# simochen/flowtrack.pytorch

Measured on AMD Instinct MI355X. Metric: pose crops/sec (ResNet-50 + 3-deconv head, 256x192), higher is better.
Workload: dtype fp16; 1 GPU; ResNet-50 pose head fp16, batch 64 x 256x192 synthetic crops per GPU (BASELINE.json configs[1]); per_gpu_batch=64, resident_batches=4, parallelism=dp1: batch sharded, one process per GPU

## Files before the change

flowtrack/pytorch_amd/_lib.py:

```python
from __future__ import annotations

import ctypes
import os
from ctypes import POINTER, c_char_p, c_double, c_float, c_int, c_int32, c_uint64, c_void_p

HERE = os.path.dirname(os.path.abspath(__file__))
LIB_PATH = os.environ.get("FT_LIB_PATH") or os.path.join(HERE, "libflowtrack_hip.so")

FT_OK = 0
FT_ERR_INVALID_ARG = 1
FT_ERR_UNSUPPORTED = 2
FT_F16, FT_F32 = 0, 1
FT_ACT_NONE, FT_ACT_RELU, FT_ACT_LEAKY = 0, 1, 2
FT_LAYOUT_NHWC, FT_LAYOUT_NCHW_F32 = 0, 1
FT_RGB_MEAN_SPLITS = 64


class FlowtrackHipError(RuntimeError):
    pass


class ConvDesc(ctypes.Structure):

    _fields_ = [
# ... 43 lines not shown
    "ft_memcpy_async": (c_int, [c_void_p, c_void_p, ctypes.c_size_t, c_void_p]),
    "ft_conv_pack_geometry": (c_int, [POINTER(ConvDesc), POINTER(ConvGeometry)]),
    "ft_conv_tile_candidates": (c_int, [POINTER(ConvDesc), POINTER(c_int), c_int]),
    "ft_conv_workspace_bytes": (ctypes.c_size_t, [POINTER(ConvDesc)]),
    "ft_conv2d_fwd_ws": (c_int, [POINTER(ConvDesc), c_void_p, c_void_p, c_void_p, c_void_p, c_void_p, c_void_p, c_void_p,
                                 ctypes.c_size_t, c_void_p]),
    "ft_conv_tap_source": (c_int, [POINTER(ConvDesc), c_int, c_int, c_int, POINTER(c_int), POINTER(c_int)]),
    "ft_conv2d_fwd": (c_int, [POINTER(ConvDesc), c_void_p, c_void_p, c_void_p, c_void_p, c_void_p,
                              c_void_p, c_void_p]),
    "ft_conv_flops": (c_double, [POINTER(ConvDesc)]),
    "ft_conv_direct_supported": (c_int, [POINTER(ConvDesc)]),
    "ft_conv_direct_stream_id": (c_int, [POINTER(ConvDesc)]),
    "ft_conv_direct_weight_bytes": (ctypes.c_longlong, [POINTER(ConvDesc)]),
    "ft_conv_direct_pack": (c_int, [POINTER(ConvDesc), c_void_p, c_int, c_int, c_void_p, c_void_p]),
    "ft_conv_direct_fwd": (c_int, [POINTER(ConvDesc), c_void_p, c_void_p, c_void_p, c_void_p, c_void_p, c_void_p, c_void_p]),
    "ft_bottleneck_supported": (c_int, [POINTER(BottleneckDesc)]),
    "ft_bottleneck_fwd": (c_int, [POINTER(BottleneckDesc), c_void_p, c_void_p, c_void_p, c_void_p, c_void_p, c_void_p, c_void_p]),
    "ft_bottleneck_flops": (c_double, [POINTER(BottleneckDesc)]),
    "ft_bottleneck_rstat_supported": (c_int, [POINTER(BottleneckDesc)]),
    "ft_bottleneck_rstat_weight_bytes": (ctypes.c_longlong, []),
    "ft_bottleneck_rstat_fwd": (c_int, [POINTER(BottleneckDesc), c_void_p, c_void_p, c_void_p, c_void_p]),
    "ft_bottleneck_stream_supported": (c_int, [POINTER(BottleneckDesc)]),
    "ft_bottleneck_stream_folds": (c_int, [POINTER(BottleneckDesc)]),
    "ft_bottleneck_stream_weight_bytes": (ctypes.c_longlong, [POINTER(BottleneckDesc)]),
    "ft_bottleneck_stream_pack": (c_int, [POINTER(BottleneckDesc), c_void_p, c_void_p, c_void_p, c_void_p, c_void_p]),
    "ft_bottleneck_stream_fwd": (c_int, [POINTER(BottleneckDesc), c_void_p, c_void_p, c_void_p, c_void_p, c_void_p]),
    "ft_pack_nchw_to_nhwc": (c_int, [c_void_p, c_void_p] + [c_int] * 8 + [c_void_p]),
    "ft_unpack_nhwc_to_nchw": (c_int, [c_void_p, c_void_p, c_int, c_int, c_int, c_int, c_int, c_int, c_int,
                                       c_void_p]),
    "ft_maxpool3x3s2_fwd": (c_int, [c_void_p, c_void_p, c_int, c_int, c_int, c_int, c_int, c_void_p]),
    "ft_bn_batch_stats": (c_int, [c_void_p, c_int, c_int, c_int, c_int, c_int, c_int, c_void_p, c_void_p, c_void_p, c_void_p]),
    "ft_heatmap_max_preds": (c_int, [c_void_p, c_int, c_int, c_int, c_int, c_int, c_void_p, c_void_p, c_void_p,
                                     c_void_p]),
    "ft_heatmap_keypoint_rows": (c_int, [c_void_p, c_int, c_int, c_int, c_int, c_int, c_void_p, c_void_p, c_void_p]),
    "ft_heatmap_min_margin": (c_int, [c_void_p, c_int, c_int, c_int, c_int, c_void_p, c_void_p]),
    "ft_heatmap_argmax_screen": (c_int, [c_void_p, c_int, c_int, c_int, c_int, c_float, c_void_p, c_void_p, c_void_p]),
    "ft_flow_rgb_mean": (c_int, [c_void_p, c_int, c_int, c_int, c_void_p, c_void_p, c_void_p]),
    "ft_flow_pack_pair": (c_int, [c_void_p, c_void_p, c_float, c_void_p] + [c_int] * 7 + [c_void_p]),
    "ft_flow_mean_pack_pair_state_words": (ctypes.c_longlong, [c_int, c_int, c_int]),
    "ft_flow_pack_pair_sums_chunks": (ctypes.c_longlong, [c_int]),
    "ft_conv_shift_nstride_supported": (c_int, [POINTER(ConvDesc)]),
    "ft_flow_pack_pair_sums": (c_int, [c_void_p, c_float, c_void_p] + [c_int] * 6 + [c_void_p, c_void_p]),
    "ft_flow_mean_fold": (c_int, [c_void_p, c_float, c_void_p] + [c_int] * 6 + [c_void_p, c_void_p, c_void_p, c_int, c_void_p, c_void_p,
                                  c_void_p]),
    "ft_flow_mean_pack_pair": (c_int, [c_void_p, c_float, c_void_p, c_int, c_int, c_void_p, c_int, c_int] + [c_int] * 4
                               + [c_void_p, c_void_p, c_void_p]),
# ... 65 lines not shown
```

flowtrack/pytorch_amd/csrc/bottleneck_stream.hip:

```cpp
#include <stdlib.h>

#include <type_traits>

#include "ft_common.h"

namespace ft {
namespace {

struct BnsParams {
  const char* x;
  char* y;
  const char* ws;
  const char* tab;
  int H, W, TH;
  int ppi, total;
  int TWc, csplit;
  int Ho, Wo;
  int x_cstride, x_coff, y_cstride, y_coff;
  unsigned x_bytes, y_bytes, ws_bytes;
  int dbg;
};

template <int N, int I = 0, typename F>
__device__ __forceinline__ void bns_unroll(F&& f) {
// ... 697 lines not shown
#pragma unroll
      for (int e = 0; e < 6; ++e)
#pragma unroll
        for (int i = 0; i < CTW; ++i)
          shp[e][i] = __builtin_amdgcn_raw_buffer_load_b32(rsrc_t, so, 4 * (e * P + (CTW * wcol + i) * 32), 0);
    } else {
#pragma unroll
      for (int t = 0; t < 48 / NW; ++t)
        __builtin_amdgcn_raw_ptr_buffer_load_lds(rsrc_t, (lds_ptr)(smem + TABS + (t * NW + wave) * 256), 4, (unsigned)lane * 4u, (t * NW + wave) * 256, 0, 0);
    }
  };
  [[maybe_unused]] auto add_shift = [&](int e, auto& A, auto mtc) {
    constexpr int MT = decltype(mtc)::value;
#pragma unroll
    for (int i = 0; i < CTW; ++i) {
      const uint4_t sa = uint4_t{shp[e][i], 0u, 0u, 0u};
#pragma unroll
      for (int j = 0; j < MT; ++j)
        A[i][j] = __builtin_amdgcn_mfma_f32_32x32x16_f16(__builtin_bit_cast(half8_t, sa), __builtin_bit_cast(half8_t, onesB), A[i][j], 0, 0, 0);
    }
  };
  issue_x(0, 0);
  load_a(std::integral_constant<int, 0>{}, 0);
  issue_touch();
  load_tables();
  asm volatile("" ::: "memory");
  issue_x(1, 1);
  issue_x(2, 2);
  bns_unroll<D - 1>([&](auto sc) { load_a(std::integral_constant<int, decltype(sc)::value + 1>{}, decltype(sc)::value + 1); });
  if (tid < ROWB / 16) *reinterpret_cast<uint4_t*>(smem + ZROW + tid * 16) = uint4_t{0u, 0u, 0u, 0u};

  uint4_t res[4][CTW][MT2][2];
  int m_out[MT2], hp_out[MT2];
#pragma unroll
  for (int j = 0; j < MT2; ++j) {
    m_out[j] = j * 32 + l31;
    if constexpr (XH) {
      const int r = m_out[j] / TWc;
      hp_out[j] = (r + 1) * PW + (m_out[j] - r * TWc) + 1;
    } else if constexpr (HEAD) {
      const int r = m_out[j] / TWc;
      hp_out[j] = (2 * r + 1) * W + 2 * (m_out[j] - r * TWc);
    } else {
      hp_out[j] = m_out[j] + W;
    }
  }

  float16_t acc1[CTW][MT1];
#pragma unroll
// ... 372 lines not shown
      zero_acc();
      if constexpr (!WSTG) {
        asm volatile("s_waitcnt lgkmcnt(0)" ::: "memory");
        BNS_BARRIER();
      } else {
        asm volatile("" ::: "memory");
      }
      readout(qc);
    });
  }
  if (p.dbg & 32) {
    ts[5] = __builtin_amdgcn_s_memtime();
    asm volatile("s_waitcnt vmcnt(0)" ::: "memory");
    ts[6] = __builtin_amdgcn_s_memtime();
    if (tid == 0) {
      unsigned long long* o = reinterpret_cast<unsigned long long*>(p.y + ((size_t)((n * p.H + y0) * W) * p.y_cstride + p.y_coff) * 2);
#pragma unroll
      for (int i = 0; i < 8; ++i) o[i] = ts[i];
    }
  }
#endif
}

template <int P>
__global__ __launch_bounds__(256) void bns_pack_kernel(const half_t* __restrict__ w1, const half_t* __restrict__ w2,
                                                       const half_t* __restrict__ w3, uint4_t* __restrict__ out) {
  using G = BnsGeom<P>;
  const int idx = blockIdx.x * 256 + threadIdx.x;
  if (idx >= G::GEND * G::WSTEP / 16) return;
  const int lane = idx & 63, frag = idx >> 6;
  const int per_step = 4 * G::NCT;
  const int g = frag / per_step, f = frag - g * per_step;
  const int kk = f / G::NCT, i = f - kk * G::NCT;
  const int l31 = lane & 31, lhi = lane >> 5;
  const int co_t = 32 * i + bns_sigma(l31);
  const int k_t = 16 * kk + 8 * lhi;
  const half_t* src;
  if (g < G::G2) {
    src = w1 + (size_t)co_t * G::C + 64 * g + k_t;
  } else if (g < G::G3) {
    const int s = g - G::G2, tap = s / G::KC, kc = s - tap * G::KC;
    src = w2 + (size_t)co_t * (9 * P) + tap * P + 64 * kc + k_t;
  } else {
    const int s = g - G::G3, q = s / G::KC, kc = s - q * G::KC;
    src = w3 + (size_t)(q * P + co_t) * P + 64 * kc + k_t;
  }
  out[idx] = *reinterpret_cast<const uint4_t*>(src);
}

__global__ __launch_bounds__(256) void bns_pack_head_kernel(const half_t* __restrict__ w1, const half_t* __restrict__ w2,
                                                            uint4_t* __restrict__ out, int C) {
  using G = BnsGeom<256>;
  const int nc1 = C / 64, gend = nc1 + 9 * G::KC;
  const int idx = blockIdx.x * 256 + threadIdx.x;
  if (idx >= gend * G::WSTEP / 16) return;
  const int lane = idx & 63, frag = idx >> 6;
  const int per_step = 4 * G::NCT;
  const int g = frag / per_step, f = frag - g * per_step;
  const int kk = f / G::NCT, i = f - kk * G::NCT;
  const int l31 = lane & 31, lhi = lane >> 5;
  const int co_t = 32 * i + bns_sigma(l31);
  const int k_t = 16 * kk + 8 * lhi;
  const half_t* src;
  if (g < nc1) {
    src = w1 + (size_t)co_t * C + 64 * g + k_t;
  } else {
    const int sft = g - nc1, tap = sft / G::KC, kc = sft - tap * G::KC;
    src = w2 + (size_t)co_t * (9 * 256) + tap * 256 + 64 * kc + k_t;
  }
  out[idx] = *reinterpret_cast<const uint4_t*>(src);
}

// ... 43 lines not shown
    auto cost = [&](int th, int mt1, int mt2) {
      const long long wg = (long long)d->N * ceil_div(d->H, th);
      return ((wg + 255) / 256) * (long long)(32 * mt1 + 104 * mt2);
    };
    bool small = th_b < 1 || (th_s >= 1 && cost(th_s, 3, 2) < cost(th_b, 4, 3));
    if (force128 == 1 && th_b >= 1) small = false;
    if (force128 == 2 && th_s >= 1) small = true;
    const int th = small ? th_s : th_b;
    *out = BnsPlan{small ? 5 : 0, th, ceil_div(d->H, th), d->W, 1};
    return FT_OK;
  }
  const int th_big = rows(96, 120), th_small = rows(64, 96);
  int xs = 0, x_tw = 0, x_th = 0;
  for (int cs = 2; cs <= 4 && !xs; ++cs) {
    const int tw = ceil_div(d->W, cs);
    int th = 32 / tw;
    const int th2 = 64 / (tw + 2) - 2;
    th = th < th2 ? th : th2;
    if (th < 1 || tw * (cs - 1) >= d->W) continue;
    th = th < d->H ? th : d->H;
    xs = cs; x_tw = tw; x_th = ceil_div(d->H, ceil_div(d->H, th));
  }
  if (th_big < 1 && th_small < 1 && !xs) return FT_ERR_UNSUPPORTED;
  int pick;
  if (force == 1 || force == 2 || (force == 3 && xs)) pick = force;
  else {
    auto cost = [&](int th, int mt1, int mt2) {
      const long long wg = (long long)d->N * ceil_div(d->H, th);
      return ((wg + 255) / 256) * (long long)(64 * mt1 + 208 * mt2);
    };
    if (th_big < 1) pick = 2;
    else if (th_small < 1) pick = 1;
    else pick = cost(th_big, 4, 3) <= cost(th_small, 3, 2) ? 1 : 2;
    if (pick == 1 && th_big < 1) pick = 2;
    if (pick == 2 && th_small < 1) pick = th_big >= 1 ? 1 : 3;
    if (xs && pick != 3) {
      const long long wgx = (long long)d->N * ceil_div(d->H, x_th) * xs;
      const long long cx = ((wgx + 255) / 256) * (long long)(64 * 2 + 208 * 1);
      const long long cf = pick == 1 ? cost(th_big, 4, 3) : cost(th_small, 3, 2);
      if (cx < cf) pick = 3;
    }
  }
  if (pick == 1 && th_big < 1) pick = 2;
  if (pick == 2 && th_small < 1) pick = th_big >= 1 ? 1 : 3;
  if (pick == 3) {
    *out = BnsPlan{3, x_th, ceil_div(d->H, x_th) * xs, x_tw, xs};
    return FT_OK;
  }
  const int th = pick == 1 ? th_big : th_small;
  *out = BnsPlan{pick, th, ceil_div(d->H, th), d->W, 1};
  return FT_OK;
}

template <int P, int MT1, int MT2, bool FOLD = false>
static int bns_launch(const BnsParams& p, hipStream_t s) {
  auto k = bottleneck_stream_kernel<P, MT1, MT2, FOLD>;
  static bool attr_done[64] = {};
  int dev = 0;
  FT_HIP_CHECK(hipGetDevice(&dev));
  if (dev < 0 || dev >= 64 || !attr_done[dev]) {
    FT_HIP_CHECK(hipFuncSetAttribute(reinterpret_cast<const void*>(k), hipFuncAttributeMaxDynamicSharedMemorySize, BnsGeom<P>::LDS_BYTES));
    if (dev >= 0 && dev < 64) attr_done[dev] = true;
  }
  hipLaunchKernelGGL(k, dim3(p.total), dim3(256), BnsGeom<P>::LDS_BYTES, s, p);
// ... 3 lines not shown

#ifndef FT_BNS_SLOTS
#define FT_BNS_SLOTS 4
#endif
#ifndef FT_BNS_XH_SLOTS
#define FT_BNS_XH_SLOTS 3
#endif
template <int MT1, int MT2, bool XH, int HEADC = 0, int NW = 4, bool FOLD = false>
static int bns_launch_direct(const BnsParams& p, hipStream_t s) {
  auto k = bottleneck_stream_direct_kernel<MT1, MT2, XH, XH ? FT_BNS_XH_SLOTS : FT_BNS_SLOTS, HEADC, NW, FOLD>;
  constexpr int lds = 81920 + 2 * MT2 * 32 * 512;
  static bool attr_done[64] = {};
  int dev = 0;
  FT_HIP_CHECK(hipGetDevice(&dev));
  if (dev < 0 || dev >= 64 || !attr_done[dev]) {
    FT_HIP_CHECK(hipFuncSetAttribute(reinterpret_cast<const void*>(k), hipFuncAttributeMaxDynamicSharedMemorySize, lds));
    if (dev >= 0 && dev < 64) attr_done[dev] = true;
  }
  hipLaunchKernelGGL(k, dim3(p.total), dim3(64 * NW), lds, s, p);
  FT_LAUNCH_CHECK("bottleneck_stream_direct_kernel");
  return FT_OK;
}

}
}

extern "C" int ft_bottleneck_stream_supported(const ft_bottleneck_desc* d) {
  ft::BnsPlan pl;
  return ft::bns_plan(d, &pl);
}

extern "C" int ft_bottleneck_stream_folds(const ft_bottleneck_desc* d) {
  ft::BnsPlan pl;
  if (ft::bns_plan(d, &pl) != FT_OK) return 0;
  return pl.variant != 4;
}

extern "C" long long ft_bottleneck_stream_weight_bytes(const ft_bottleneck_desc* d) {
  ft::BnsPlan pl;
  if (ft::bns_plan(d, &pl) != FT_OK) return 0;
  if (pl.variant == 4) return (long long)(d->C / 64 + 9 * ft::BnsGeom<256>::KC) * ft::BnsGeom<256>::WSTEP;
  return d->P == 128 ? (long long)ft::BnsGeom<128>::GEND * ft::BnsGeom<128>::WSTEP : (long long)ft::BnsGeom<256>::GEND * ft::BnsGeom<256>::WSTEP;
}

extern "C" int ft_bottleneck_stream_pack(const ft_bottleneck_desc* d, const void* w1, const void* w2, const void* w3, void* wstream,
                                         ft_stream_t stream) {
  using namespace ft;
  BnsPlan pl;
  const int st = bns_plan(d, &pl);
  if (st != FT_OK) return st;
  if (!w1 || !w2 || (!w3 && pl.variant != 4) || !wstream) return FT_ERR_INVALID_ARG;
  hipStream_t s = as_stream(stream);
  const half_t *a = static_cast<const half_t*>(w1), *b = static_cast<const half_t*>(w2), *c = static_cast<const half_t*>(w3);
  if (pl.variant == 4) {
    const int n16 = (int)(ft_bottleneck_stream_weight_bytes(d) / 16);
    hipLaunchKernelGGL(bns_pack_head_kernel, dim3(ceil_div(n16, 256)), dim3(256), 0, s, a, b, static_cast<uint4_t*>(wstream), d->C);
    FT_LAUNCH_CHECK("bns_pack_head_kernel");
    return FT_OK;
  }
  if (d->P == 128) {
    const int n16 = BnsGeom<128>::GEND * BnsGeom<128>::WSTEP / 16;
    hipLaunchKernelGGL(bns_pack_kernel<128>, dim3(ceil_div(n16, 256)), dim3(256), 0, s, a, b, c, static_cast<uint4_t*>(wstream));
  } else {
    const int n16 = BnsGeom<256>::GEND * BnsGeom<256>::WSTEP / 16;
    hipLaunchKernelGGL(bns_pack_kernel<256>, dim3(ceil_div(n16, 256)), dim3(256), 0, s, a, b, c, static_cast<uint4_t*>(wstream));
  }
  FT_LAUNCH_CHECK("bns_pack_kernel");
  return FT_OK;
}

extern "C" int ft_bottleneck_stream_fwd(const ft_bottleneck_desc* d, const void* x, const void* wstream, const float* tables, void* y,
                                        ft_stream_t stream) {
  using namespace ft;
  BnsPlan pl;
  const int st = bns_plan(d, &pl);
  if (st != FT_OK) return st;
  if (!x || !wstream || !tables || !y || x == y) return FT_ERR_INVALID_ARG;
  if (d->folded && pl.variant == 4) return FT_ERR_UNSUPPORTED;
  BnsParams p{};
  p.x = static_cast<const char*>(x);
  p.y = static_cast<char*>(y);
  p.ws = static_cast<const char*>(wstream);
  p.tab = reinterpret_cast<const char*>(tables);
  p.H = d->H; p.W = d->W; p.TH = pl.TH; p.ppi = pl.ppi;
  p.TWc = pl.TWc; p.csplit = pl.csplit;
  if (pl.variant == 4) { p.Ho = d->H / 2; p.Wo = d->W / 2; }
  p.total = d->N * pl.ppi;
  p.x_cstride = d->x_cstride; p.x_coff = d->x_coff; p.y_cstride = d->y_cstride; p.y_coff = d->y_coff;
  p.x_bytes = (unsigned)((size_t)d->N * d->H * d->W * d->x_cstride * 2);
  p.y_bytes = (unsigned)((size_t)d->N * d->H * d->W * d->y_cstride * 2);
  p.ws_bytes = (unsigned)ft_bottleneck_stream_weight_bytes(d);
  if (pl.variant == 4) p.y_bytes = (unsigned)((size_t)d->N * p.Ho * p.Wo * d->y_cstride * 2);
  static const int dbg = dev_env_int("FT_BNS_DBG", 0);
  p.dbg = dbg;
  if (dbg & 64) p.ws_bytes = 0;
  if (dbg & 128) p.x_bytes = 0;
  hipStream_t s = as_stream(stream);
  const bool waves8 = dev_env_int("FT_BNS_WAVES", pl.variant == 3 ? 8 : 4) == 8;
  if (d->folded) {
    switch (pl.variant) {
      case 0: return bns_launch<128, 4, 3, true>(p, s);
      case 5: return bns_launch<128, 3, 2, true>(p, s);
      case 1: return bns_launch<256, 4, 3, true>(p, s);
      case 3: return waves8 ? bns_launch_direct<2, 1, true, 0, 8, true>(p, s) : bns_launch_direct<2, 1, true, 0, 4, true>(p, s);
      default: return waves8 ? bns_launch_direct<3, 2, false, 0, 8, true>(p, s) : bns_launch_direct<3, 2, false, 0, 4, true>(p, s);
    }
  }
  switch (pl.variant) {
    case 0: return bns_launch<128, 4, 3>(p, s);
    case 5: return bns_launch<128, 3, 2>(p, s);
    case 1: return bns_launch<256, 4, 3>(p, s);
    case 3: return waves8 ? bns_launch_direct<2, 1, true, 0, 8>(p, s) : bns_launch_direct<2, 1, true>(p, s);
    case 4: return waves8 ? bns_launch_direct<4, 1, false, 8, 8>(p, s) : bns_launch_direct<4, 1, false, 8>(p, s);
    default:
      return waves8 ? bns_launch_direct<3, 2, false, 0, 8>(p, s) : bns_launch_direct<3, 2, false>(p, s);
  }
}
```

flowtrack/pytorch_amd/csrc/ft_common.h:

```cpp
#pragma once
#include <hip/hip_runtime.h>
#include <stdint.h>
#include <stdlib.h>

#include "flowtrack_hip.h"

namespace ft {

int record_hip_error(hipError_t e, const char* what);

#define FT_HIP_CHECK(expr)                                         \
  do {                                                             \
    hipError_t _e = (expr);                                        \
    if (_e != hipSuccess) return ::ft::record_hip_error(_e, #expr); \
  } while (0)

#define FT_LAUNCH_CHECK(name)                                        \
  do {                                                               \
    hipError_t _e = hipGetLastError();                               \
    if (_e != hipSuccess) return ::ft::record_hip_error(_e, name);   \
  } while (0)

#define FT_RAISE_LDS(kernel, bytes)                                                                              \
  do {                                                                                                           \
// ... 51 lines not shown
  }
}
__device__ __forceinline__ half8_t bn_res_relu_acc8(const float16_t& acc, int h, const float4_t (&sc)[4], const float4_t (&sh)[4], const half8_t& rs) {
  half8_t o;
#pragma unroll
  for (int e = 0; e < 8; e += 2) {
    const int r = h * 8 + e;
    const half2_t v = bn_res_relu_pk(acc[r], acc[r + 1], sc[r >> 2][r & 3], sc[r >> 2][(r & 3) + 1], sh[r >> 2][r & 3], sh[r >> 2][(r & 3) + 1], rs[e], rs[e + 1]);
    o[e] = v[0];
    o[e + 1] = v[1];
  }
  return o;
}

__device__ __forceinline__ void relu_acc16(const float16_t& acc, half8_t (&h8)[2]) {
#pragma unroll
  for (int r = 0; r < 16; r += 2) {
    const half2_t o = __builtin_elementwise_max(__builtin_convertvector(float2_t{acc[r], acc[r + 1]}, half2_t), half2_t{(half_t)0.f, (half_t)0.f});
    h8[r >> 3][r & 7] = o[0];
    h8[r >> 3][(r & 7) + 1] = o[1];
  }
}

#ifndef FT_YSTORE_AUX
#define FT_YSTORE_AUX 16
#endif
#define FT_YSTORE_BUF_AUX (FT_YSTORE_AUX == 2 ? 2 : ((FT_YSTORE_AUX & 16) ? FT_YSTORE_AUX : 0))
__device__ __forceinline__ void store_out16(void* ptr, uint4_t v) {
#if FT_YSTORE_AUX == 16
  asm volatile("global_store_dwordx4 %0, %1, off sc1\n\ts_nop 1" ::"v"(ptr), "v"(v) : "memory");
#elif FT_YSTORE_AUX == 17
  asm volatile("global_store_dwordx4 %0, %1, off sc0 sc1\n\ts_nop 1" ::"v"(ptr), "v"(v) : "memory");
#elif FT_YSTORE_AUX == 2
  __builtin_nontemporal_store(v, reinterpret_cast<uint4_t*>(ptr));
#else
  *reinterpret_cast<uint4_t*>(ptr) = v;
#endif
}

}
```

flowtrack/pytorch_amd/hip_ops.py:

```python
from __future__ import annotations

import ctypes
import functools
import json
import os
import sys
from dataclasses import dataclass
from typing import List, Optional, Sequence, Tuple

import torch

from . import _lib
from ._lib import (FT_ACT_LEAKY, FT_ACT_NONE, FT_ACT_RELU, FT_LAYOUT_NCHW_F32, FT_LAYOUT_NHWC,
                   ConvDesc, ConvGeometry, FlowtrackHipError, check)

ACT_CODES = {None: FT_ACT_NONE, "none": FT_ACT_NONE, "relu": FT_ACT_RELU, "leaky": FT_ACT_LEAKY}


def require_gpu(device: torch.device) -> None:
    if device.type != "cuda" or not torch.cuda.is_available():
        raise FlowtrackHipError(
            "the flowtrack HIP path needs a ROCm GPU (model.cuda()); there is no CPU fallback — "
            "use oracle/ for CPU reference results")

# ... 1018 lines not shown
    if scale is not None:
        w = w * scale[:, None]
    return w.half().contiguous(), (shift if shift is not None else torch.zeros(conv.cout))


def _fold_representable(convs) -> bool:
    for c in convs:
        w, sh = _folded_kmajor(c)
        if not bool(torch.isfinite(w.float()).all()) or not bool(torch.isfinite(sh.float().half().float()).all()):
            return False
    return True


def shift_pairs(shift: torch.Tensor) -> torch.Tensor:
    hi = shift.float().half()
    lo = (shift.float() - hi.float()).half()
    return torch.stack([hi, lo], dim=-1).contiguous().view(torch.int32).reshape(-1)


def _bottleneck_stream_operands(c1: "FusedConv", d, x: ActView, planes: int, p1, p2, p3, convs=None):
    lib = _lib.load()
    (w1, s1, b1), (w2, s2, b2), (w3, s3, b3) = p1, p2, p3
    folded = convs is not None
    key = ("bns_stream_folded" if folded else "bns_stream", x.N, x.H, x.W)
    cached = c1._packed.get(key) if hasattr(c1, "_packed") else None
    if cached is None:
        P = planes
        if folded:
            dev = x.t.device
            (w1, sh1), (w2, sh2), (w3, sh3) = (_folded_kmajor(c) for c in convs)
            if (tuple(w1.shape), tuple(w2.shape), tuple(w3.shape)) != ((P, 4 * P), (P, 9 * P), (4 * P, P)):
                raise FlowtrackHipError(f"folded bottleneck weights: unexpected shapes {tuple(w1.shape)} {tuple(w2.shape)} {tuple(w3.shape)}")
            w1, w2, w3 = w1.to(dev), w2.to(dev), w3.to(dev)
            tables = torch.cat([shift_pairs(sh1), shift_pairs(sh2), shift_pairs(sh3)]).contiguous().to(dev)
        else:
            tables = torch.cat([s1.flatten()[:P], b1.flatten()[:P], s2.flatten()[:P], b2.flatten()[:P]] +
                               [t.flatten()[q * P:(q + 1) * P] for q in range(4) for t in (s3, b3)]).float().contiguous()
        nbytes = int(lib.ft_bottleneck_stream_weight_bytes(ctypes.byref(d)))
        wstream = torch.empty(nbytes, dtype=torch.uint8, device=x.t.device)
        check(lib.ft_bottleneck_stream_pack(ctypes.byref(d), w1.data_ptr(), w2.data_ptr(), w3.data_ptr(), wstream.data_ptr(),
                                            current_stream_handle(x.t.device)), "ft_bottleneck_stream_pack")
        torch.cuda.current_stream(x.t.device).synchronize()
        cached = (wstream, tables)
        if hasattr(c1, "_packed"):
            c1._packed[key] = cached
    return cached

# ... 146 lines not shown
```

include/flowtrack_hip.h:

```cpp
#ifndef FLOWTRACK_HIP_H_
#define FLOWTRACK_HIP_H_

#include <stddef.h>
#include <stdint.h>

#ifdef __cplusplus
extern "C" {
#endif

enum {
  FT_OK = 0,
  FT_ERR_INVALID_ARG = 1,
  FT_ERR_UNSUPPORTED = 2,
  FT_ERR_HIP = 3,
  FT_ERR_NO_DEVICE = 4
};

enum { FT_F16 = 0, FT_F32 = 1 };
enum { FT_ACT_NONE = 0, FT_ACT_RELU = 1, FT_ACT_LEAKY = 2 };
enum { FT_LAYOUT_NHWC = 0, FT_LAYOUT_NCHW_F32 = 1 };

typedef void* ft_stream_t;

int ft_version(void);
// ... 70 lines not shown
int ft_conv_direct_pack(const ft_conv_desc* d, const void* w_packed, int kpad, int cout_pad, void* wstream, ft_stream_t stream);
int ft_conv_direct_fwd(const ft_conv_desc* d, const void* x, const void* wstream, const float* scale, const float* shift,
                       const void* residual, void* y, ft_stream_t stream);

typedef struct ft_bottleneck_desc {
  int dtype;
  int N, H, W;
  int C, P;
  int x_cstride, x_coff;
  int y_cstride, y_coff;
  int head_only;
  int projection;
  int stride;
  int folded;
} ft_bottleneck_desc;
int ft_bottleneck_supported(const ft_bottleneck_desc* d);
int ft_bottleneck_fwd(const ft_bottleneck_desc* d, const void* x,
                      const void* w1, const void* w2, const void* w3,
                      const float* scale_shift, void* y, ft_stream_t stream);
double ft_bottleneck_flops(const ft_bottleneck_desc* d);

int ft_bottleneck_stream_supported(const ft_bottleneck_desc* d);
int ft_bottleneck_stream_folds(const ft_bottleneck_desc* d);
long long ft_bottleneck_stream_weight_bytes(const ft_bottleneck_desc* d);
int ft_bottleneck_stream_pack(const ft_bottleneck_desc* d, const void* w1, const void* w2, const void* w3, void* wstream,
                              ft_stream_t stream);
int ft_bottleneck_stream_fwd(const ft_bottleneck_desc* d, const void* x, const void* wstream, const float* tables, void* y,
                             ft_stream_t stream);

int ft_pack_nchw_to_nhwc(const float* x, void* y, int N, int C, int H, int W,
                         int cpad, int lpad, int wpitch, int dtype,
                         ft_stream_t stream);
int ft_unpack_nhwc_to_nchw(const void* x, float* y, int N, int C, int H, int W,
                           int x_cstride, int x_coff, int dtype,
                           ft_stream_t stream);
int ft_maxpool3x3s2_fwd(const void* x, void* y, int N, int Hi, int Wi, int C,
                        int dtype, ft_stream_t stream);

int ft_bn_batch_stats(const void* x, int N, int H, int W, int C, int x_cstride, int dtype,
                      float* workspace, float* mean, float* var, ft_stream_t stream);

int ft_heatmap_max_preds(const float* heatmaps, int N, int K, int H, int W,
                         int adjust_coords, int32_t* idx, float* score,
                         float* coords, ft_stream_t stream);
int ft_heatmap_keypoint_rows(const float* heatmaps, int N, int K, int H, int W,
                             int adjust_coords, int32_t* idx, float* rows,
// ... 99 lines not shown
```

Baseline: 56140 crops/s.

## Add 16x16 MFMA tile variant of fused bottleneck stream kernel for P=256

Adds a new fused bottleneck kernel variant for P=256 folded blocks that uses 16x16x32 MFMA tiles with smaller pixel tiles (48-80 rows-worth), plus a matching weight-pack kernel and a packed-weight layout key so cached weights match the chosen variant. The planner picks this variant when its estimated wave cost beats the existing 32x32 variants, aiming to reduce tile-quantization waste and improve workgroup balance on the late ResNet stage. It also inserts scheduling barriers around the prologue loads in the existing kernel. The new path adds register/LDS pressure (launch bounds 1) and relies on a heuristic cost model that may misjudge.

```diff
diff --git a/flowtrack/pytorch_amd/_lib.py b/flowtrack/pytorch_amd/_lib.py
--- a/flowtrack/pytorch_amd/_lib.py
+++ b/flowtrack/pytorch_amd/_lib.py
@@ -89,6 +89,7 @@
     "ft_bottleneck_rstat_fwd": (c_int, [POINTER(BottleneckDesc), c_void_p, c_void_p, c_void_p, c_void_p]),
     "ft_bottleneck_stream_supported": (c_int, [POINTER(BottleneckDesc)]),
     "ft_bottleneck_stream_folds": (c_int, [POINTER(BottleneckDesc)]),
+    "ft_bottleneck_stream_layout": (c_int, [POINTER(BottleneckDesc)]),
     "ft_bottleneck_stream_weight_bytes": (ctypes.c_longlong, [POINTER(BottleneckDesc)]),
     "ft_bottleneck_stream_pack": (c_int, [POINTER(BottleneckDesc), c_void_p, c_void_p, c_void_p, c_void_p, c_void_p]),
     "ft_bottleneck_stream_fwd": (c_int, [POINTER(BottleneckDesc), c_void_p, c_void_p, c_void_p, c_void_p, c_void_p]),
diff --git a/flowtrack/pytorch_amd/csrc/bottleneck_stream.hip b/flowtrack/pytorch_amd/csrc/bottleneck_stream.hip
--- a/flowtrack/pytorch_amd/csrc/bottleneck_stream.hip
+++ b/flowtrack/pytorch_amd/csrc/bottleneck_stream.hip
@@ -743,9 +743,12 @@
   };
   issue_x(0, 0);
   load_a(std::integral_constant<int, 0>{}, 0);
+  asm volatile("" ::: "memory");
+  __builtin_amdgcn_sched_barrier(0);
   issue_touch();
   load_tables();
   asm volatile("" ::: "memory");
+  __builtin_amdgcn_sched_barrier(0);
   issue_x(1, 1);
   issue_x(2, 2);
   bns_unroll<D - 1>([&](auto sc) { load_a(std::integral_constant<int, decltype(sc)::value + 1>{}, decltype(sc)::value + 1); });
@@ -1164,6 +1167,414 @@
 #endif
 }
 
+template <int NS>
+__global__ __launch_bounds__(256, 1) void bottleneck_stream_tile16_kernel(const BnsParams p) {
+#if defined(__HIP_DEVICE_COMPILE__)
+  constexpr int P = 256;
+  using G = BnsGeom<P>;
+  constexpr int NC1 = G::NC1, KC = G::KC, WSTEP = G::WSTEP, ROWB = G::ROWB;
+  constexpr int G2 = NC1, G3 = G2 + 9 * KC, GEND = G3 + 4 * KC;
+  constexpr int CT = 4, MT1 = 5, MT2 = 3, NT = 256;
+  constexpr int LX = (MT1 * 2 + 3) / 4;
+  constexpr int NOUT = MT2 * 16;
+  constexpr int ZROW = 61440, TOUCH = 77824, STG = 81920, STGB = 4 * NOUT * 128;
+  static_assert(LX * 4 * 8 * 128 <= G::XSTRIDE && MT1 * 16 * ROWB <= ZROW && STG + 2 * STGB <= 163840, "LDS map");
+  extern __shared__ __attribute__((aligned(16))) char smem[];
+  typedef __attribute__((address_space(3))) void* lds_ptr;
+  using c0 = std::integral_constant<int, 0>;
+  using c1 = std::integral_constant<int, 1>;
+  const int tid = threadIdx.x, lane = tid & 63;
+  const int wave = __builtin_amdgcn_readfirstlane(tid >> 6);
+  const int l15 = lane & 15, lq = lane >> 4;
+
+  int logical;
+  {
+    const int b = blockIdx.x;
+    const int q = p.total >> 3, r = p.total & 7, xcd = b & 7, loc = b >> 3;
+    logical = (xcd < r ? xcd * (q + 1) : r * (q + 1) + (xcd - r) * q) + loc;
+  }
+  const int n = logical / p.ppi;
+  const int W = p.W;
+  const int y0 = (logical - n * p.ppi) * p.TH;
+  const int rows_out = p.H - y0 < p.TH ? p.H - y0 : p.TH;
+  const int npix_out = rows_out * W;
+  const int npix_halo = (p.TH + 2) * W;
+  const int iy0 = y0 - 1;
+
+  const __amdgpu_buffer_rsrc_t rsrc_x = __builtin_amdgcn_make_buffer_rsrc(const_cast<char*>(p.x), 0, p.x_bytes, 0x00020000);
+  const __amdgpu_buffer_rsrc_t rsrc_y = __builtin_amdgcn_make_buffer_rsrc(p.y, 0, p.y_bytes, 0x00020000);
+  const __amdgpu_buffer_rsrc_t rsrc_w = __builtin_amdgcn_make_buffer_rsrc(const_cast<char*>(p.ws), 0, p.ws_bytes, 0x00020000);
+  const __amdgpu_buffer_rsrc_t rsrc_t = __builtin_amdgcn_make_buffer_rsrc(const_cast<char*>(p.tab), 0, (2 * P + G::C) * 4, 0x00020000);
+  constexpr unsigned kOOB = 0x80000000u;
+
+  unsigned x_voff[LX];
+#pragma unroll
+  for (int t = 0; t < LX; ++t) {
+    const int hp = (t * 4 + wave) * 8 + (lane >> 3);
+    const int hr = hp / W, hc = hp - hr * W;
+    const int iy = iy0 + hr;
+    unsigned v = kOOB;
+    if (hp < npix_halo && (unsigned)iy < (unsigned)p.H)
+      v = (unsigned)((((n * p.H + iy) * W + hc) * p.x_cstride + p.x_coff) * 2 + (((lane & 7) ^ BNS_XKEY(hp)) << 4));
+    x_voff[t] = v;
+  }
+  const unsigned lane16 = (unsigned)lane * 16u;
+  auto issue_x = [&](int c, int buf) {
+    char* dst = smem + buf * G::XSTRIDE;
+#pragma unroll
+    for (int t = 0; t < LX; ++t)
+      __builtin_amdgcn_raw_ptr_buffer_load_lds(rsrc_x, (lds_ptr)(dst + (t * 4 + wave) * 1024), 16, x_voff[t], c * 128, 0, 0);
+  };
+  static_assert(NS >= 3 && 12 % NS == 0, "ring phase of the unrolled phase-2 body (12 steps per kernel row)");
+  constexpr int D = NS - 1;
+  uint4_t areg[NS][2][CT];
+  auto load_a_slice = [&](auto slotc, int g, auto ksc) {
+    constexpr int SL = decltype(slotc)::value, ks = decltype(ksc)::value;
+#pragma unroll
+    for (int t = 0; t < CT; ++t)
+      areg[SL][ks][t] = __builtin_amdgcn_raw_buffer_load_b128(rsrc_w, lane16, g * WSTEP + (ks * 16 + CT * wave + t) * 1024, 0);
+  };
+  auto load_a = [&](auto slotc, int g) {
+    load_a_slice(slotc, g, c0{});
+    load_a_slice(slotc, g, c1{});
+  };
+  unsigned long long ts[8] = {0, 0, 0, 0, 0, 0, 0, 0};
+  BNSD_TS(0);
+  constexpr int kTouch = 6;
+  auto issue_touch = [&]() {
+    const bool on = blockIdx.x < 256 && !(p.dbg & 512);
+    const int xcd = blockIdx.x & 7, loc = blockIdx.x >> 3;
+    const int first = p.total < 256 ? p.total : 256;
+    const int nloc = (first - xcd + 7) >> 3;
+    const unsigned lines = (p.ws_bytes + 127u) >> 7;
+    const unsigned per = (lines + nloc - 1) / nloc;
+    const unsigned lo = loc * per, hi = lo + per < lines ? lo + per : lines;
+#pragma unroll
+    for (int k = 0; k < kTouch; ++k) {
+      const unsigned l = lo + tid + (unsigned)(NT * k);
+      __builtin_amdgcn_raw_ptr_buffer_load_lds(rsrc_w, (lds_ptr)(smem + TOUCH + wave * 256), 4, (on && l < hi) ? l << 7 : kOOB, 0, 0, 0);
+    }
+  };
+  unsigned shp[6][CT];
+  uint4_t permA[2];
+  const uint4_t onesB = uint4_t{0x3C003C00u, 0u, 0u, 0u};
+  {
+    const bool on = lq == (l15 >> 2);
+#pragma unroll
+    for (int o = 0; o < 2; ++o) {
+      const int pe = 4 * o + (l15 & 3);
+      unsigned w[4];
+#pragma unroll
+      for (int k = 0; k < 4; ++k) w[k] = (on && (pe >> 1) == k) ? (0x3C00u << (16 * (pe & 1))) : 0u;
+      permA[o] = uint4_t{w[0], w[1], w[2], w[3]};
+    }
+  }
+  constexpr int kTabLoads = 2 * CT;
+  auto load_tables = [&](int e0, int e1) {
+    const unsigned so = lq == 0 ? 4u * (unsigned)(16 * (l15 >> 2) + (l15 & 3)) : kOOB;
+#pragma unroll
+    for (int e = e0; e < e1; ++e)
+#pragma unroll
+      for (int t = 0; t < CT; ++t)
+        shp[e][t] = __builtin_amdgcn_raw_buffer_load_b32(rsrc_t, so, 4 * (e * P + 64 * wave + 4 * t), 0);
+  };
+  auto add_shift = [&](int e, auto& A, auto mtc) {
+    constexpr int MT = decltype(mtc)::value;
+#pragma unroll
+    for (int t = 0; t < CT; ++t) {
+      const uint4_t sa = uint4_t{shp[e][t], 0u, 0u, 0u};
+#pragma unroll
+      for (int j = 0; j < MT; ++j)
+        A[t][j] = __builtin_amdgcn_mfma_f32_16x16x32_f16(__builtin_bit_cast(half8_t, sa), __builtin_bit_cast(half8_t, onesB), A[t][j], 0, 0, 0);
+    }
+  };
+  issue_x(0, 0);
+  load_a(c0{}, 0);
+  asm volatile("" ::: "memory");
+  __builtin_amdgcn_sched_barrier(0);
+  issue_touch();
+  load_tables(0, 2);
+  asm volatile("" ::: "memory");
+  __builtin_amdgcn_sched_barrier(0);
+  issue_x(1, 1);
+  issue_x(2, 2);
+  bns_unroll<D - 1>([&](auto sc) { load_a(std::integral_constant<int, decltype(sc)::value + 1>{}, decltype(sc)::value + 1); });
+  if (tid < ROWB / 16) *reinterpret_cast<uint4_t*>(smem + ZROW + tid * 16) = uint4_t{0u, 0u, 0u, 0u};
+
+  uint4_t res[4][MT2][2];
+  int m_out[MT2], hp_out[MT2];
+#pragma unroll
+  for (int j = 0; j < MT2; ++j) {
+    m_out[j] = j * 16 + l15;
+    hp_out[j] = m_out[j] + W;
+  }
+
+  float4_t acc1[CT][MT1];
+#pragma unroll
+  for (int t = 0; t < CT; ++t)
+#pragma unroll
+    for (int j = 0; j < MT1; ++j) acc1[t][j] = float4_t{0.f, 0.f, 0.f, 0.f};
+  int b1_off[MT1];
+#pragma unroll
+  for (int j = 0; j < MT1; ++j) {
+    const int hp = j * 16 + l15;
+    b1_off[j] = hp * 128 + ((lq ^ BNS_XKEY(hp)) << 4);
+  }
+  {
+    uint4_t fx[2][MT1];
+    auto ldx = [&](auto setc, int buf, int ks) {
+      constexpr int S = decltype(setc)::value;
+      const char* xb = smem + buf * G::XSTRIDE;
+#pragma unroll
+      for (int j = 0; j < MT1; ++j) fx[S][j] = *reinterpret_cast<const uint4_t*>(xb + (b1_off[j] ^ (ks << 6)));
+    };
+    auto mma1 = [&](auto setc, auto slotc, auto ksc) {
+      constexpr int S = decltype(setc)::value, SL = decltype(slotc)::value, ks = decltype(ksc)::value;
+#pragma unroll
+      for (int j = 0; j < MT1; ++j)
+#pragma unroll
+        for (int t = 0; t < CT; ++t)
+          acc1[t][j] = __builtin_amdgcn_mfma_f32_16x16x32_f16(__builtin_bit_cast(half8_t, areg[SL][ks][t]),
+                                                              __builtin_bit_cast(half8_t, fx[S][j]), acc1[t][j], 0, 0, 0);
+    };
+    static_assert(2 * LX + 2 * CT * D + kTouch + kTabLoads <= 63, "vmcnt immediate");
+    asm volatile("s_waitcnt vmcnt(%0) lgkmcnt(0)" ::"n"(2 * LX + 2 * CT * D + kTouch + kTabLoads) : "memory");
+    BNS_BARRIER();
+    BNSD_TS(7);
+    ldx(c0{}, 0, 0);
+    bns_unroll<NC1>([&](auto cc) {
+      constexpr int c = decltype(cc)::value;
+      constexpr int buf = c % 3;
+      using slot = std::integral_constant<int, c % NS>;
+      using nslot = std::integral_constant<int, (c + D) % NS>;
+      load_a_slice(nslot{}, c + D, c0{});
+      ldx(c1{}, buf, 1);
+      mma1(c0{}, slot{}, c0{});
+      __builtin_amdgcn_sched_group_barrier(0x020, LX, 0);
+      bns_unroll<MT1>([&](auto) {
+        __builtin_amdgcn_sched_group_barrier(0x100, 1, 0);
+        __builtin_amdgcn_sched_group_barrier(0x008, 2, 0);
+      });
+      bns_unroll<CT>([&](auto) {
+        __builtin_amdgcn_sched_group_barrier(0x020, 1, 0);
+        __builtin_amdgcn_sched_group_barrier(0x008, 2, 0);
+      });
+      __builtin_amdgcn_sched_group_barrier(0x008, CT * MT1 - 2 * MT1 - 2 * CT, 0);
+      bns_unroll<MT1>([&](auto) {
+        __builtin_amdgcn_sched_group_barrier(0x100, 1, 0);
+        __builtin_amdgcn_sched_group_barrier(0x008, 2, 0);
+      });
+      if (c % 4 == wave) {
+        constexpr int q = c / 4;
+        const char* xb = smem + buf * G::XSTRIDE;
+#pragma unroll
+        for (int j = 0; j < MT2; ++j) {
+          const int hp = hp_out[j];
+          const char* rowp = xb + hp * 128;
+#pragma unroll
+          for (int h = 0; h < 2; ++h)
+            res[q][j][h] = *reinterpret_cast<const uint4_t*>(rowp + (((2 * lq + h) ^ BNS_XKEY(hp)) << 4));
+        }
+      }
+      load_a_slice(nslot{}, c + D, c1{});
+      if constexpr (c + 1 < NC1) {
+        if constexpr (c + 2 < NC1) asm volatile("s_waitcnt vmcnt(%0) lgkmcnt(0)" ::"n"(LX + 4 * CT) : "memory");
+        else asm volatile("s_waitcnt vmcnt(%0) lgkmcnt(0)" ::"n"(4 * CT) : "memory");
+        BNS_BARRIER();
+        if constexpr (c + 3 < NC1) issue_x(c + 3, buf);
+        ldx(c0{}, (c + 1) % 3, 0);
+      }
+      mma1(c1{}, slot{}, c1{});
+    });
+  }
+  BNSD_TS(1);
+  asm volatile("s_waitcnt lgkmcnt(0)" ::: "memory");
+  BNS_BARRIER();
+  auto pieces = [&](auto& A, int j, half8_t (&h8)[2]) {
+    h8[0] = relu_acc4x2(A[0][j], A[1][j]);
+    h8[1] = relu_acc4x2(A[2][j], A[3][j]);
+  };
+  {
+    add_shift(0, acc1, std::integral_constant<int, MT1>{});
+#pragma unroll
+    for (int j = 0; j < MT1; ++j) {
+      const int hp = j * 16 + l15;
+      const int iy = iy0 + hp / W;
+      const bool inside = (unsigned)iy < (unsigned)p.H;
+      half8_t h8[2];
+      pieces(acc1, j, h8);
+#pragma unroll
+      for (int h = 0; h < 2; ++h) {
+        uint4_t u = __builtin_bit_cast(uint4_t, h8[h]);
+        u.x = inside ? u.x : 0u; u.y = inside ? u.y : 0u; u.z = inside ? u.z : 0u; u.w = inside ? u.w : 0u;
+        h8[h] = __builtin_bit_cast(half8_t, u);
+      }
+      if (hp < npix_halo) {
+        char* rowp = smem + hp * ROWB;
+        const int cb = wave * 8 + 2 * lq;
+#pragma unroll
+        for (int h = 0; h < 2; ++h) *reinterpret_cast<half8_t*>(rowp + (((cb + h) ^ (hp & 15)) << 4)) = h8[h];
+      }
+    }
+  }
+  asm volatile("s_waitcnt lgkmcnt(0)" ::: "memory");
+  BNS_BARRIER();
+  BNSD_TS(2);
+  load_tables(2, 6);
+
+  float4_t acc[CT][MT2];
+  auto zero_acc = [&]() {
+#pragma unroll
+    for (int t = 0; t < CT; ++t)
+#pragma unroll
+      for (int j = 0; j < MT2; ++j) acc[t][j] = float4_t{0.f, 0.f, 0.f, 0.f};
+  };
+  zero_acc();
+  int edge[MT2];
+#pragma unroll
+  for (int j = 0; j < MT2; ++j) {
+    const int ox = m_out[j] % W;
+    edge[j] = (ox == 0 ? 1 : 0) | (ox == W - 1 ? 2 : 0);
+  }
+  auto row_bases = [&](int off, int kc, int bad, int (&rb)[MT2]) {
+#pragma unroll
+    for (int j = 0; j < MT2; ++j) {
+      const int row = m_out[j] + off;
+      const int v = row * ROWB + (((row & 15) ^ lq) << 4);
+      rb[j] = ((edge[j] & bad) ? ZROW + (lq << 4) : v) ^ (kc << 7);
+    }
+  };
+  uint4_t fb[2][MT2];
+  auto ldb = [&](auto setc, int ks, const int (&rb)[MT2]) {
+    constexpr int S = decltype(setc)::value;
+#pragma unroll
+    for (int j = 0; j < MT2; ++j) fb[S][j] = *reinterpret_cast<const uint4_t*>(smem + (rb[j] ^ (ks << 6)));
+  };
+  auto mma2 = [&](auto setc, auto slotc, auto ksc) {
+    constexpr int S = decltype(setc)::value, SL = decltype(slotc)::value, ks = decltype(ksc)::value;
+#pragma unroll
+    for (int j = 0; j < MT2; ++j)
+#pragma unroll
+      for (int t = 0; t < CT; ++t)
+        acc[t][j] = __builtin_amdgcn_mfma_f32_16x16x32_f16(__builtin_bit_cast(half8_t, areg[SL][ks][t]),
+                                                           __builtin_bit_cast(half8_t, fb[S][j]), acc[t][j], 0, 0, 0);
+  };
+  auto dstep = [&](auto slotc, int g, const int (&rb)[MT2], bool has_next, const int (&rbn)[MT2]) {
+    constexpr int SL = decltype(slotc)::value;
+    using slot = std::integral_constant<int, SL>;
+    load_a(std::integral_constant<int, (SL + D) % NS>{}, g + D);
+    ldb(c1{}, 1, rb);
+    mma2(c0{}, slot{}, c0{});
+    if (has_next) ldb(c0{}, 0, rbn);
+    mma2(c1{}, slot{}, c1{});
+    bns_unroll<8>([&](auto ic) {
+      constexpr int i = decltype(ic)::value;
+      __builtin_amdgcn_sched_group_barrier(0x100, (i & 3) < MT2 ? 1 : 0, 0);
+      __builtin_amdgcn_sched_group_barrier(0x008, CT * MT2 / 4, 0);
+      __builtin_amdgcn_sched_group_barrier(0x020, 1, 0);
+    });
+  };
+
+  {
+    static_assert((3 * KC) % NS == 0, "ring phase of the unrolled body");
+    int rb[MT2], rbn[MT2];
+    row_bases(-1, 0, 1, rb);
+    ldb(c0{}, 0, rb);
+    for (int ky = 0; ky < 3; ++ky) {
+      bns_unroll<3 * KC>([&](auto sc) {
+        constexpr int s = decltype(sc)::value;
+        constexpr int kx = s / KC, kc = s % KC;
+        constexpr int nkc = (kc + 1) % KC, nkx = kc + 1 == KC ? (kx + 1) % 3 : kx;
+        const int nky = (kc + 1 == KC && kx == 2) ? ky + 1 : ky;
+        row_bases(nky * W + nkx - 1, nkc, nkx == 0 ? 1 : (nkx == 2 ? 2 : 0), rbn);
+        dstep(std::integral_constant<int, (G2 + s) % NS>{}, G2 + 3 * KC * ky + s, rb, true, rbn);
+#pragma unroll
+        for (int j = 0; j < MT2; ++j) rb[j] = rbn[j];
+      });
+    }
+  }
+  BNSD_TS(3);
+  asm volatile("s_waitcnt lgkmcnt(0)" ::: "memory");
+  BNS_BARRIER();
+  {
+    add_shift(1, acc, std::integral_constant<int, MT2>{});
+#pragma unroll
+    for (int j = 0; j < MT2; ++j) {
+      const int m = m_out[j];
+      half8_t h8[2];
+      pieces(acc, j, h8);
+      char* rowp = smem + m * ROWB;
+      const int cb = wave * 8 + 2 * lq;
+#pragma unroll
+      for (int h = 0; h < 2; ++h) *reinterpret_cast<half8_t*>(rowp + (((cb + h) ^ (m & 15)) << 4)) = h8[h];
+    }
+  }
+  zero_acc();
+  asm volatile("s_waitcnt lgkmcnt(0)" ::: "memory");
+  BNS_BARRIER();
+  BNSD_TS(4);
+
+  {
+    constexpr int NSTG = NOUT / 8;
+    unsigned s_voff[NSTG];
+    int s_off[NSTG];
+#pragma unroll
+    for (int k = 0; k < NSTG; ++k) {
+      const int m = (lane >> 3) + 8 * k, ch = lane & 7;
+      s_voff[k] = m < npix_out ? (unsigned)((((n * p.H + y0) * W + m) * p.y_cstride + p.y_coff + wave * 64 + ch * 8) * 2) : kOOB;
+      s_off[k] = wave * (NOUT * 128) + m * 128 + ((ch ^ (m & 7)) << 4);
+    }
+    int rb[MT2], rbn[MT2];
+    row_bases(0, 0, 0, rb);
+    ldb(c0{}, 0, rb);
+    bns_unroll<4>([&](auto qc) {
+      constexpr int q = decltype(qc)::value;
+      bns_unroll<KC>([&](auto kcc) {
+        constexpr int kc = decltype(kcc)::value;
+        constexpr int g = G3 + q * KC + kc;
+        row_bases(0, (kc + 1) % KC, 0, rbn);
+        dstep(std::integral_constant<int, g % NS>{}, g, rb, g + 1 < GEND, rbn);
+#pragma unroll
+        for (int j = 0; j < MT2; ++j) rb[j] = rbn[j];
+      });
+      add_shift(2 + q, acc, std::integral_constant<int, MT2>{});
+#pragma unroll
+      for (int t = 0; t < CT; ++t)
+#pragma unroll
+        for (int j = 0; j < MT2; ++j)
+          acc[t][j] = __builtin_amdgcn_mfma_f32_16x16x32_f16(__builtin_bit_cast(half8_t, permA[t & 1]),
+                                                             __builtin_bit_cast(half8_t, res[q][j][t >> 1]), acc[t][j], 0, 0, 0);
+      char* stg = smem + STG + (q & 1) * STGB + wave * (NOUT * 128);
+#pragma unroll
+      for (int j = 0; j < MT2; ++j) {
+        const int m = m_out[j];
+        half8_t h8[2];
+        pieces(acc, j, h8);
+#pragma unroll
+        for (int h = 0; h < 2; ++h) *reinterpret_cast<half8_t*>(stg + m * 128 + (((2 * lq + h) ^ (m & 7)) << 4)) = h8[h];
+      }
+      zero_acc();
+      asm volatile("" ::: "memory");
+#pragma unroll
+      for (int k = 0; k < NSTG; ++k) {
+        const uint4_t v = *reinterpret_cast<const uint4_t*>(smem + STG + (q & 1) * STGB + s_off[k]);
+        if (!(p.dbg & 4)) __builtin_amdgcn_raw_buffer_store_b128(v, rsrc_y, s_voff[k] + (unsigned)(q * P * 2), 0, FT_YSTORE_BUF_AUX);
+      }
+    });
+  }
+  if (p.dbg & 32) {
+    ts[5] = __builtin_amdgcn_s_memtime();
+    asm volatile("s_waitcnt vmcnt(0)" ::: "memory");
+    ts[6] = __builtin_amdgcn_s_memtime();
+    if (tid == 0) {
+      unsigned long long* o = reinterpret_cast<unsigned long long*>(p.y + ((size_t)((n * p.H + y0) * W) * p.y_cstride + p.y_coff) * 2);
+#pragma unroll
+      for (int i = 0; i < 8; ++i) o[i] = ts[i];
+    }
+  }
+#endif
+}
+
 template <int P>
 __global__ __launch_bounds__(256) void bns_pack_kernel(const half_t* __restrict__ w1, const half_t* __restrict__ w2,
                                                        const half_t* __restrict__ w3, uint4_t* __restrict__ out) {
@@ -1190,6 +1601,31 @@
   out[idx] = *reinterpret_cast<const uint4_t*>(src);
 }
 
+__global__ __launch_bounds__(256) void bns_pack16_kernel(const half_t* __restrict__ w1, const half_t* __restrict__ w2,
+                                                         const half_t* __restrict__ w3, uint4_t* __restrict__ out) {
+  using G = BnsGeom<256>;
+  constexpr int P = 256;
+  const int idx = blockIdx.x * 256 + threadIdx.x;
+  if (idx >= G::GEND * G::WSTEP / 16) return;
+  const int lane = idx & 63, frag = idx >> 6;
+  const int g = frag >> 5, f = frag & 31;
+  const int ks = f >> 4, t = f & 15;
+  const int r = lane & 15;
+  const int co_t = 64 * (t >> 2) + 16 * (r >> 2) + 4 * (t & 3) + (r & 3);
+  const int k_t = 32 * ks + 8 * (lane >> 4);
+  const half_t* src;
+  if (g < G::G2) {
+    src = w1 + (size_t)co_t * G::C + 64 * g + k_t;
+  } else if (g < G::G3) {
+    const int s = g - G::G2, tap = s / G::KC, kc = s - tap * G::KC;
+    src = w2 + (size_t)co_t * (9 * P) + tap * P + 64 * kc + k_t;
+  } else {
+    const int s = g - G::G3, q = s / G::KC, kc = s - q * G::KC;
+    src = w3 + (size_t)(q * P + co_t) * P + 64 * kc + k_t;
+  }
+  out[idx] = *reinterpret_cast<const uint4_t*>(src);
+}
+
 __global__ __launch_bounds__(256) void bns_pack_head_kernel(const half_t* __restrict__ w1, const half_t* __restrict__ w2,
                                                             uint4_t* __restrict__ out, int C) {
   using G = BnsGeom<256>;
@@ -1279,8 +1715,9 @@
     xs = cs; x_tw = tw; x_th = ceil_div(d->H, ceil_div(d->H, th));
   }
   if (th_big < 1 && th_small < 1 && !xs) return FT_ERR_UNSUPPORTED;
+  const int th_16 = d->folded ? rows(48, 80) : 0;
   int pick;
-  if (force == 1 || force == 2 || (force == 3 && xs)) pick = force;
+  if (force == 1 || force == 2 || (force == 3 && xs) || (force == 6 && th_16 >= 1)) pick = force;
   else {
     auto cost = [&](int th, int mt1, int mt2) {
       const long long wg = (long long)d->N * ceil_div(d->H, th);
@@ -1291,12 +1728,21 @@
     else pick = cost(th_big, 4, 3) <= cost(th_small, 3, 2) ? 1 : 2;
     if (pick == 1 && th_big < 1) pick = 2;
     if (pick == 2 && th_small < 1) pick = th_big >= 1 ? 1 : 3;
+    long long cf = pick == 1 ? cost(th_big, 4, 3) : (pick == 2 ? cost(th_small, 3, 2) : -1);
+    if (th_16 >= 1 && dev_env_int("FT_BNS_WAVES", 4) != 8) {
+      const long long wg = (long long)d->N * ceil_div(d->H, th_16);
+      const long long c16 = ((wg + 255) / 256) * (long long)(32 * 5 + 104 * 3);
+      if (cf < 0 || c16 < cf) { pick = 6; cf = c16; }
+    }
     if (xs && pick != 3) {
       const long long wgx = (long long)d->N * ceil_div(d->H, x_th) * xs;
       const long long cx = ((wgx + 255) / 256) * (long long)(64 * 2 + 208 * 1);
-      const long long cf = pick == 1 ? cost(th_big, 4, 3) : cost(th_small, 3, 2);
       if (cx < cf) pick = 3;
     }
+  }
+  if (pick == 6) {
+    *out = BnsPlan{6, th_16, ceil_div(d->H, th_16), d->W, 1};
+    return FT_OK;
   }
   if (pick == 1 && th_big < 1) pick = 2;
   if (pick == 2 && th_small < 1) pick = th_big >= 1 ? 1 : 3;
@@ -1346,6 +1792,15 @@
   return FT_OK;
 }
 
+static int bns_launch_tile16(const BnsParams& p, hipStream_t s) {
+  auto k = bottleneck_stream_tile16_kernel<FT_BNS_SLOTS>;
+  constexpr int lds = 81920 + 2 * 4 * 48 * 128;
+  FT_RAISE_LDS(k, lds);
+  hipLaunchKernelGGL(k, dim3(p.total), dim3(256), lds, s, p);
+  FT_LAUNCH_CHECK("bottleneck_stream_tile16_kernel");
+  return FT_OK;
+}
+
 }
 }
 
@@ -1358,6 +1813,12 @@
   ft::BnsPlan pl;
   if (ft::bns_plan(d, &pl) != FT_OK) return 0;
   return pl.variant != 4;
+}
+
+extern "C" int ft_bottleneck_stream_layout(const ft_bottleneck_desc* d) {
+  ft::BnsPlan pl;
+  if (ft::bns_plan(d, &pl) != FT_OK) return -1;
+  return pl.variant == 6 ? 1 : 0;
 }
 
 extern "C" long long ft_bottleneck_stream_weight_bytes(const ft_bottleneck_desc* d) {
@@ -1385,6 +1846,9 @@
   if (d->P == 128) {
     const int n16 = BnsGeom<128>::GEND * BnsGeom<128>::WSTEP / 16;
     hipLaunchKernelGGL(bns_pack_kernel<128>, dim3(ceil_div(n16, 256)), dim3(256), 0, s, a, b, c, static_cast<uint4_t*>(wstream));
+  } else if (pl.variant == 6) {
+    const int n16 = BnsGeom<256>::GEND * BnsGeom<256>::WSTEP / 16;
+    hipLaunchKernelGGL(bns_pack16_kernel, dim3(ceil_div(n16, 256)), dim3(256), 0, s, a, b, c, static_cast<uint4_t*>(wstream));
   } else {
     const int n16 = BnsGeom<256>::GEND * BnsGeom<256>::WSTEP / 16;
     hipLaunchKernelGGL(bns_pack_kernel<256>, dim3(ceil_div(n16, 256)), dim3(256), 0, s, a, b, c, static_cast<uint4_t*>(wstream));
@@ -1426,6 +1890,7 @@
       case 0: return bns_launch<128, 4, 3, true>(p, s);
       case 5: return bns_launch<128, 3, 2, true>(p, s);
       case 1: return bns_launch<256, 4, 3, true>(p, s);
+      case 6: return bns_launch_tile16(p, s);
       case 3: return waves8 ? bns_launch_direct<2, 1, true, 0, 8, true>(p, s) : bns_launch_direct<2, 1, true, 0, 4, true>(p, s);
       default: return waves8 ? bns_launch_direct<3, 2, false, 0, 8, true>(p, s) : bns_launch_direct<3, 2, false, 0, 4, true>(p, s);
     }
diff --git a/flowtrack/pytorch_amd/csrc/ft_common.h b/flowtrack/pytorch_amd/csrc/ft_common.h
--- a/flowtrack/pytorch_amd/csrc/ft_common.h
+++ b/flowtrack/pytorch_amd/csrc/ft_common.h
@@ -97,6 +97,18 @@
   }
 }
 
+__device__ __forceinline__ half8_t relu_acc4x2(const float4_t& a, const float4_t& b) {
+  half8_t o;
+#pragma unroll
+  for (int r = 0; r < 4; r += 2) {
+    const half2_t u = __builtin_elementwise_max(__builtin_convertvector(float2_t{a[r], a[r + 1]}, half2_t), half2_t{(half_t)0.f, (half_t)0.f});
+    const half2_t v = __builtin_elementwise_max(__builtin_convertvector(float2_t{b[r], b[r + 1]}, half2_t), half2_t{(half_t)0.f, (half_t)0.f});
+    o[r] = u[0]; o[r + 1] = u[1];
+    o[4 + r] = v[0]; o[4 + r + 1] = v[1];
+  }
+  return o;
+}
+
 #ifndef FT_YSTORE_AUX
 #define FT_YSTORE_AUX 16
 #endif
diff --git a/flowtrack/pytorch_amd/hip_ops.py b/flowtrack/pytorch_amd/hip_ops.py
--- a/flowtrack/pytorch_amd/hip_ops.py
+++ b/flowtrack/pytorch_amd/hip_ops.py
@@ -1064,7 +1064,8 @@
     lib = _lib.load()
     (w1, s1, b1), (w2, s2, b2), (w3, s3, b3) = p1, p2, p3
     folded = convs is not None
-    key = ("bns_stream_folded" if folded else "bns_stream", x.N, x.H, x.W)
+    layout = int(lib.ft_bottleneck_stream_layout(ctypes.byref(d)))
+    key = ("bns_stream_folded" if folded else "bns_stream", x.N, x.H, x.W, layout)
     cached = c1._packed.get(key) if hasattr(c1, "_packed") else None
     if cached is None:
         P = planes
diff --git a/include/flowtrack_hip.h b/include/flowtrack_hip.h
--- a/include/flowtrack_hip.h
+++ b/include/flowtrack_hip.h
@@ -116,6 +116,7 @@
 
 int ft_bottleneck_stream_supported(const ft_bottleneck_desc* d);
 int ft_bottleneck_stream_folds(const ft_bottleneck_desc* d);
+int ft_bottleneck_stream_layout(const ft_bottleneck_desc* d);
 long long ft_bottleneck_stream_weight_bytes(const ft_bottleneck_desc* d);
 int ft_bottleneck_stream_pack(const ft_bottleneck_desc* d, const void* w1, const void* w2, const void* w3, void* wstream,
                               ft_stream_t stream);
```

Result: faster. 57140 crops/s, median of 6 (+1.8%).
